# sbyrnes321/metalens

Hardware: AMD Instinct MI355X
Metric: aperture x far-field pair-evals/sec (higher is better)
Workload: dtype f64; 1 GPU; 1 mm dia NA=0.5 lens, lambda=580 nm, 4096x4096 aperture window at pitch lambda/2.2 -> 512x512 far-field directions (bins of the aperture FFT lattice x 1), fp64, on-axis x-dipole at the focus; aperture=4096, farfield=512, rings=197, centre_cells=1219855, orders=survey, pmc_key=gpus=1,aperture=4096,farfield=512,precision=f64,method=auto,zoom=1,pols=1, pmc_stale=True

## Files before the change

### metalens_amd/csrc/nearfield_simple.hip

```cpp
#include <algorithm>
#include <type_traits>

#include "nearfield_math.h"
#include "synth_staging.h"

namespace ml {


#ifdef __HIP_DEVICE_COMPILE__
#define ML_GLOBAL __attribute__((address_space(1)))
#else
#define ML_GLOBAL
#endif
struct Consts {
    double kvac, kvac2, kg2, efh, sx, sy, dz, dz2, z2;
    double b0, b1, b2, b3;
    const ML_GLOBAL double2 *ring_rec, *rot_table, *ring_tab, *premod;
    const ML_GLOBAL int2 *geo_ix;
    ML_GLOBAL double *fields, *partial_power;
    int plane_wave, patches_x, n_rings, outside_is_zero, nx, ny, n_partials;
    double hcoef, pcoef, pol[3];
};
template <bool FIXED3>
__device__ __forceinline__ void load_consts(const NfArgs &a, Consts &K) {
    K.kvac = a.p.kvac;
    K.kvac2 = a.p.kvac2;
    K.kg2 = a.p.k_glass2;
    K.efh = a.e_from_h;
    K.sx = a.p.source_x;
    K.sy = a.p.source_y;
    K.dz = a.p.dz;
    K.dz2 = a.p.dz2;
    K.z2 = a.p.source_z2;
    K.ring_rec = (const ML_GLOBAL double2 *)a.ring_rec;
    K.rot_table = (const ML_GLOBAL double2 *)a.rot_table;
    K.ring_tab = (const ML_GLOBAL double2 *)a.ring_tab;
    K.plane_wave = FIXED3 ? 0 : a.p.plane_wave;
    K.b0 = a.ring_bounds_all[0];
    K.b1 = a.ring_bounds_all[1];
    K.b2 = a.ring_bounds_all[2];
    K.b3 = a.ring_bounds_all[3];
    K.premod = FIXED3 ? nullptr : (const ML_GLOBAL double2 *)a.premod;
    K.geo_ix = (const ML_GLOBAL int2 *)a.geo_ix;
    K.fields = (ML_GLOBAL double *)a.fields;
    K.patches_x = a.patches_x;
    K.n_rings = a.n_rings;
    K.outside_is_zero = a.outside_is_zero;
    K.nx = a.nx;
    K.ny = a.ny;
    if (FIXED3)
        asm volatile("" : "+s"(K.kvac), "+s"(K.kvac2), "+s"(K.kg2), "+s"(K.efh), "+s"(K.sx), "+s"(K.sy), "+s"(K.dz), "+s"(K.dz2),
                     "+s"(K.z2), "+s"(K.ring_rec), "+s"(K.rot_table), "+s"(K.ring_tab));
    else
        asm volatile("" : "+s"(K.kvac), "+s"(K.kvac2), "+s"(K.kg2), "+s"(K.efh), "+s"(K.sx), "+s"(K.sy), "+s"(K.dz), "+s"(K.dz2),
                     "+s"(K.z2), "+s"(K.ring_rec), "+s"(K.rot_table), "+s"(K.ring_tab), "+s"(K.plane_wave));
    K.partial_power = (ML_GLOBAL double *)a.partial_power;
    K.n_partials = a.n_partials;
    K.hcoef = a.hcoef[0];
    K.pcoef = a.pcoef[0];
    K.pol[0] = a.pol[0][0];
    K.pol[1] = a.pol[0][1];
    K.pol[2] = a.pol[0][2];
    if (FIXED3)
        asm volatile("" : "+s"(K.b0), "+s"(K.b1), "+s"(K.b2), "+s"(K.b3), "+s"(K.geo_ix), "+s"(K.fields),
                     "+s"(K.patches_x), "+s"(K.n_rings), "+s"(K.outside_is_zero), "+s"(K.nx), "+s"(K.ny));
    else
        asm volatile("" : "+s"(K.b0), "+s"(K.b1), "+s"(K.b2), "+s"(K.b3), "+s"(K.premod), "+s"(K.geo_ix), "+s"(K.fields),
                     "+s"(K.patches_x), "+s"(K.n_rings), "+s"(K.outside_is_zero), "+s"(K.nx), "+s"(K.ny));
    asm volatile("" : "+s"(K.partial_power), "+s"(K.n_partials), "+s"(K.hcoef), "+s"(K.pcoef), "+s"(K.pol[0]), "+s"(K.pol[1]),
                 "+s"(K.pol[2]));
}

__device__ __forceinline__ void wave_power_k(const NfArgs &a, const Consts &K, double power_here, int bx, int by, int member) {
    power_here = dpp_add<0x111, 0xf>(power_here);
    power_here = dpp_add<0x112, 0xf>(power_here);
    power_here = dpp_add<0x114, 0xf>(power_here);
    power_here = dpp_add<0x118, 0xf>(power_here);
    const int lane = threadIdx.x & 63;
    if ((lane & 15) == 15)
        K.partial_power[(size_t)member * K.n_partials + ((size_t)by * K.patches_x + bx) * 4 + (lane >> 4)] = power_here;
    if (blockIdx.x == 0 && blockIdx.y == 0 && member == 0)
        for (int k = threadIdx.x; k < a.n_viol_keys; k += 64) a.viol_next[k] = 0ull;
}

struct AccS {
    double Exr, Exi, Eyr, Eyi, Hxr, Hxi, Hyr, Hyi;
};

struct OrderShared {
    double kx0, G, ky, ky2;
    c2 E0, X;
};

struct OrderFactors {
    double cxy, cxx, cyy;
    c2 ph;
};

__device__ __forceinline__ double small_int_as_double(int ox) {
    const unsigned m = (unsigned)(ox < 0 ? -ox : ox);
    unsigned hi = m ? 0x3ff00000u + (((0x98640u >> (4 * (m - 1))) & 15u) << 18) : 0u;
    hi |= ox < 0 ? 0x80000000u : 0u;
    return __longlong_as_double((long long)((unsigned long long)hi << 32));
}

struct OrderWalk {
    c2 ph;
    double kx;
};
__device__ __forceinline__ void walk_start(OrderWalk &w, const OrderShared &S, int lo) {
    w.ph = S.E0;
#pragma nounroll
    for (int l = lo; l < 0; ++l) w.ph = cmulf_conj(w.ph, S.X);
#pragma nounroll
    for (int l = 0; l < lo; ++l) w.ph = cmulf(w.ph, S.X);
    w.kx = fma(small_int_as_double(lo), S.G, S.kx0);
}
__device__ __forceinline__ void walk_step(OrderWalk &w, const OrderShared &S) {
    w.ph = cmulf(w.ph, S.X);
    w.kx += S.G;
}

__device__ __forceinline__ bool order_setup(const OrderShared &S, const Consts &K, double kx, double &kt2) {
    kt2 = kx * kx + S.ky2;
    return kt2 <= K.kvac2;
}
__device__ __forceinline__ void order_factors_s(OrderFactors &f, const OrderShared &S, const Consts &K, const OrderWalk &w,
                                                double kt2) {
    const double g = K.efh * rsqrt_fast(K.kg2 - kt2);
    f.cxy = (w.kx * S.ky) * g;
    f.cxx = (K.kg2 - w.kx * w.kx) * g;
    f.cyy = (S.ky2 - K.kg2) * g;
    f.ph = w.ph;
}

__device__ __forceinline__ void order_accumulate(AccS &acc, const OrderFactors &f, double ufy_r, double ufy_i,
                                                 double ufx_r, double ufx_i) {
    const double vy_r = fma(ufy_r, f.ph.r, -(ufy_i * f.ph.i)), vy_i = fma(ufy_r, f.ph.i, ufy_i * f.ph.r);
    const double vx_r = fma(ufx_r, f.ph.r, -(ufx_i * f.ph.i)), vx_i = fma(ufx_r, f.ph.i, ufx_i * f.ph.r);
    acc.Hxr += vy_r;
    acc.Hxi += vy_i;
    acc.Hyr += vx_r;
    acc.Hyi += vx_i;
    acc.Exr = fma(f.cxx, vx_r, fma(f.cxy, vy_r, acc.Exr));
    acc.Exi = fma(f.cxx, vx_i, fma(f.cxy, vy_i, acc.Exi));
    acc.Eyr = fma(-f.cxy, vx_r, fma(f.cyy, vy_r, acc.Eyr));
    acc.Eyi = fma(-f.cxy, vx_i, fma(f.cyy, vy_i, acc.Eyi));
}

template <int NP, int STRIDE>
__device__ __forceinline__ void order_simple(AccS *acc, const double2 *blk, const double *wa, const double *wb,
                                             const double *Hwx, const double *Hwy, const OrderShared &S,
                                             const Consts &K, const OrderWalk &w, bool mine) {
    double kt2;
    if (!((int)order_setup(S, K, w.kx, kt2) & (int)mine)) return;
    OrderFactors f;
    order_factors_s(f, S, K, w, kt2);
    if (NP == 1) {
        double ufy_r, ufy_i, ufx_r, ufx_i;
#pragma unroll
        for (int c = 0; c < 4; ++c) {
            const double2 v0 = blk[(c * 4 + 0) * STRIDE], v1 = blk[(c * 4 + 1) * STRIDE];
            const double2 v2 = blk[(c * 4 + 2) * STRIDE], v3 = blk[(c * 4 + 3) * STRIDE];
            if (c == 0) {
                ufy_r = wa[0] * v0.x;
                ufy_i = wa[0] * v0.y;
                ufx_r = wa[0] * v1.x;
                ufx_i = wa[0] * v1.y;
            } else {
                ufy_r = fma(wa[c], v0.x, ufy_r);
                ufy_i = fma(wa[c], v0.y, ufy_i);
                ufx_r = fma(wa[c], v1.x, ufx_r);
                ufx_i = fma(wa[c], v1.y, ufx_i);
            }
            ufy_r = fma(wb[c], v2.x, ufy_r);
            ufy_i = fma(wb[c], v2.y, ufy_i);
            ufx_r = fma(wb[c], v3.x, ufx_r);
            ufx_i = fma(wb[c], v3.y, ufx_i);
            if (c == 1) __builtin_amdgcn_sched_barrier(0);
        }
        order_accumulate(acc[0], f, ufy_r, ufy_i, ufx_r, ufx_i);
    } else {
        double ar[4], ai[4];
#pragma unroll
        for (int c = 0; c < 4; ++c)
#pragma unroll
            for (int q = 0; q < 4; ++q) {
                const double2 v = blk[(c * 4 + q) * STRIDE];
                ar[q] = c == 0 ? wa[0] * v.x : fma(wa[c], v.x, ar[q]);
                ai[q] = c == 0 ? wa[0] * v.y : fma(wa[c], v.y, ai[q]);
            }
#pragma unroll
        for (int m = 0; m < NP; ++m)
            order_accumulate(acc[m], f, fma(Hwx[m], ar[0], Hwy[m] * ar[2]), fma(Hwx[m], ai[0], Hwy[m] * ai[2]),
                             fma(Hwx[m], ar[1], Hwy[m] * ar[3]), fma(Hwx[m], ai[1], Hwy[m] * ai[3]));
    }
}

__device__ __forceinline__ void locate_uniform(const double *ax, double lim0, double lim1, double u, double v,
                                               int &i0, double &t0, int &i1, double &t1) {
    const double a0 = (u - ax[0]) * ax[2], a1 = (v - ax[3]) * ax[5];
    const double f0 = fmin(fmax(floor(a0), 0.0), lim0), f1 = fmin(fmax(floor(a1), 0.0), lim1);
    i0 = (int)f0;
    i1 = (int)f1;
    t0 = a0 - f0;
    t1 = a1 - f1;
}

__device__ __forceinline__ void locate_axis(const double *axis, int n, double x, int &i, double &t) {
    i = 0;
    for (int a = 1; a < n - 1; ++a) i = (axis[a] <= x) ? a : i;
    const double lo = axis[i], hi = axis[i + 1];
    t = (x - lo) * recip(hi - lo);
}

template <bool RING>
__device__ __forceinline__ void report_orders(const NfArgs &a, double kvac2, double kx0, double G, double ky, int n_slots,
                                              int lo, unsigned present, int slot, double u, double v, double period) {
    const TableDesc &T = RING ? a.tables[slot] : a.center_desc;
    const double ky2 = ky * ky;
    for (int oc = 0; oc < n_slots; ++oc) {
        if (!((present >> oc) & 1u)) continue;
        const double kx = fma((double)(lo + oc), G, kx0);
        if (kx * kx + ky2 <= kvac2) check_bounds(a, T, slot, __popc(present & ((1u << oc) - 1u)), u, v, period, RING);
    }
}

__device__ __forceinline__ void store_fields_k(const Consts &K, int member, int i, int j, c2 Ex, c2 Ey, c2 Hx, c2 Hy) {
    const size_t plane = (size_t)K.nx * K.ny;
    const size_t at = (size_t)i * K.ny + j;
    typedef double double2v __attribute__((ext_vector_type(2)));
    double2v *F = reinterpret_cast<double2v *>(K.fields) + (size_t)member * 4 * plane;
    __builtin_nontemporal_store((double2v){Ex.r, Ex.i}, F + at);
    __builtin_nontemporal_store((double2v){Ey.r, Ey.i}, F + plane + at);
    __builtin_nontemporal_store((double2v){Hx.r, Hx.i}, F + 2 * plane + at);
    __builtin_nontemporal_store((double2v){Hy.r, Hy.i}, F + 3 * plane + at);
}

__device__ __forceinline__ void incidence(const Consts &K, double x, double y, double &ux, double &uy, double &uz,
                                          double &inv) {
    const double dx = x - K.sx, dy = y - K.sy;
    inv = rsqrt_fast(fma(dx, dx, fma(dy, dy, K.dz2)));
    ux = dx * inv;
    uy = dy * inv;
    uz = K.dz * inv;
}

__device__ __forceinline__ void rotate_dir(double ux, double uy, double2 cs, double &uxp, double &uyp) {
    uxp = fma(ux, cs.x, uy * cs.y);
    uyp = fma(uy, cs.x, -(ux * cs.y));
}

__device__ __forceinline__ unsigned lds_address(const double2 *p) {
    return (unsigned)(__UINTPTR_TYPE__)(__attribute__((address_space(3))) const char *)(const char *)p;
}
#pragma clang diagnostic push
#pragma clang diagnostic ignored "-Winline-asm"
template <int N16>
__device__ __forceinline__ void stage_block(const double2 *src, const double2 *lds, unsigned lane_off) {
    const char *base = reinterpret_cast<const char *>(src);
    const unsigned dst = lds_address(lds);
#pragma unroll
    for (int m = 0; m < N16; ++m)
        asm volatile("s_mov_b32 m0, %2\n\ts_nop 0\n\tglobal_load_lds_dwordx4 %0, %1"
                     :
                     : "v"(lane_off), "s"(base + m * 1024), "s"(dst + m * 1024)
                     : "memory", "m0");
}
#pragma clang diagnostic pop

template <int LEFT>
__device__ __forceinline__ void staged_wait() {
    asm volatile("s_waitcnt vmcnt(%0)" ::"n"(LEFT) : "memory");
}

constexpr int CB = CENTER_BLOCK;

typedef int int2v __attribute__((ext_vector_type(2)));

#ifdef ML_PHASE_TIMERS
constexpr int PHASE_SLOTS = 10, PHASE_WAVES = 1 << 18;
__device__ unsigned long long g_phase[(size_t)PHASE_SLOTS * PHASE_WAVES];
#define ML_MARK(k, dep)                                   \
    do {                                                  \
        asm volatile("" ::"v"(dep));                      \
        __builtin_amdgcn_sched_barrier(0);                \
        stamp[k] = __builtin_amdgcn_s_memtime();          \
        __builtin_amdgcn_sched_barrier(0);                \
    } while (0)
#else
#define ML_MARK(k, dep)
#endif

enum { PART_RING = 1, PART_CENTRE = 2 };
#ifndef ML_NF_PRIO
#define ML_NF_PRIO 1
#endif
#define ML_PRIO_AT(point, level)                                                                                          \
    do {                                                                                                                  \
        if (PART == PART_RING && NP == 1 && LISTED && ML_NF_PRIO == 1 && ((point) == 0 || (point) == 2))                  \
            __builtin_amdgcn_s_setprio(level);                                                                            \
    } while (0)
#ifndef ML_NF_KEEP_ROT
#define ML_NF_KEEP_ROT 0
#endif

constexpr int FIXED3_SLOTS = 3, FIXED3_PRESENT = 7;
static_assert(narrow_pitch(FIXED3_SLOTS) == 49 && narrow_cap(narrow_pitch(FIXED3_SLOTS)) == SK_SLOTS_NARROW && FIXED3_SLOTS * UNIT == 48,
              "the fixed-shape ring kernel's pitch, capacity and staging lanes");
template <int NP, int PART, bool LISTED, bool WIDE, bool FIXED3 = false>
__device__ __forceinline__ void synthesize_patch(const NfArgs &a, double2 *s_tab, double2 *s_tab1, int bx, int by) {
    static_assert(!FIXED3 || (NP == 1 && LISTED && !WIDE), "fixed-shape kernels: one source, from the lists, narrow");
    const int lane = threadIdx.x;
    const unsigned lane_off = (unsigned)lane * 16u;
    ML_PRIO_AT(0, 3);
    Consts K;
    load_consts<FIXED3>(a, K);
    const int i = by * 8 + (lane >> 3);
    const int j = bx * 8 + (lane & 7);
    const bool inb = j < K.ny && i < K.nx;
    const double x = a.x_pts[min(i, K.nx - 1)], y = a.y_pts[min(j, K.ny - 1)];
    const int2v ix = reinterpret_cast<const int2v *>(K.geo_ix + ((size_t)by * K.patches_x + bx) * 64)[lane];
#ifdef ML_PHASE_TIMERS
    unsigned long long stamp[PHASE_SLOTS] = {0};
    stamp[0] = __builtin_amdgcn_s_memtime();
    struct StampOut {
        unsigned long long *st;
        size_t wid;
        __device__ ~StampOut() {
            st[7] = __builtin_amdgcn_s_memtime();
            __builtin_amdgcn_s_waitcnt(0);
            st[8] = __builtin_amdgcn_s_memtime();
            if (threadIdx.x == 0 && wid < PHASE_WAVES && PART == PART_RING)
                for (int k = 0; k < PHASE_SLOTS; ++k) g_phase[wid * PHASE_SLOTS + k] = st[k];
        }
    } stamp_out{stamp, (size_t)by * K.patches_x + bx};
#endif
    double ux = 0.0, uy = 0.0, uz = 1.0;
    double Hx_i[NP], Hy_i[NP], power_in[NP];
    if (K.plane_wave) {
#pragma unroll
        for (int m = 0; m < NP; ++m) {
            Hx_i[m] = a.pw_Hx[m];
            Hy_i[m] = a.pw_Hy[m];
            power_in[m] = a.pw_power[m];
        }
    } else {
        double inv;
        incidence(K, x, y, ux, uy, uz, inv);
        const double t = uz * inv, rs = rsqrt_fast(uz);
        const double t2 = t * t;
#pragma unroll
        for (int m = 0; m < NP; ++m) {
            const double *pol = NP == 1 ? K.pol : a.pol[m];
            const double amp = ((NP == 1 ? K.hcoef : a.hcoef[m]) * rs) * t;
            const double hx = fma(uy, pol[2], -(uz * pol[1]));
            const double hy = fma(uz, pol[0], -(ux * pol[2]));
            const double hz = fma(ux, pol[1], -(uy * pol[0]));
            Hx_i[m] = hx * amp;
            Hy_i[m] = hy * amp;
            power_in[m] = ((NP == 1 ? K.pcoef : a.pcoef[m]) * t2) * fma(hx, hx, fma(hy, hy, hz * hz));
        }
    }
    int idx = inb ? ix.x : K.n_rings + 1;
    const int aux = inb ? ix.y : -1;
    ML_MARK(1, idx + aux);
    const int cell_type = idx >> REC_TYPE_SHIFT;
    idx &= (1 << REC_TYPE_SHIFT) - 1;
    const bool lens = idx <= K.n_rings;
    const bool peri_any = lens && idx >= 1;
    const bool peri = PART == PART_RING ? peri_any && (((WIDE ? a.wide_mask : a.narrow_mask) >> cell_type) & 1) != 0 : peri_any;
    const bool mine_too = PART == PART_RING ? (!WIDE || !a.narrow_exists || (LISTED && !a.first_pass && !__ballot(peri_any && ((a.narrow_mask >> cell_type) & 1))))
                                            : (LISTED && (FIXED3 || !a.first_pass) && !__ballot(peri_any));
    if (mine_too) {
#pragma unroll
        for (int m = 0; m < NP; ++m) wave_power_k(a, K, lens ? power_in[m] : 0.0, bx, by, m);
        if (!LISTED && inb && !lens && !K.outside_is_zero) {
            const c2 zero = {0.0, 0.0};
#pragma unroll
            for (int m = 0; m < NP; ++m) store_fields_k(K, m, i, j, zero, zero, zero, zero);
        }
    }
    ML_MARK(2, Hx_i[0]);

    if (PART == PART_CENTRE) {
        if (!__ballot(lens && !peri_any)) return;
    const bool cen = lens && !peri_any && aux >= 0;
    AccS acc[NP];
#pragma unroll
    for (int m = 0; m < NP; ++m) acc[m] = {0, 0, 0, 0, 0, 0, 0, 0};
    const TableDesc &T = a.center_desc;
    int i0, i1;
    double t0, t1;
    if (FIXED3 || T.uniform) {
        locate_uniform(T.uni_ax, (double)(T.n0 - 2), (double)(T.n1 - 2), ux, uy, i0, t0, i1, t1);
    } else {
        locate_axis(T.axis0, T.n0, ux, i0, t0);
        locate_axis(T.axis1, T.n1, uy, i1, t1);
    }
    const bool out_c = (int)(ux < T.bounds[0]) | (int)(ux > T.bounds[1]) | (int)(uy < T.bounds[2]) |
                       (int)(uy > T.bounds[3]);
    const int n2 = T.n2, groups = (n2 + SK_TYPES - 1) / SK_TYPES;
    const int which = min(cell_type, n2 - 1);
    const int grp = which / SK_TYPES;
    const int cblk = (i0 * (T.n1 - 1) + i1) * groups + grp;
    const size_t order_blocks = (size_t)(T.n0 - 1) * (T.n1 - 1) * groups;
    const int n_slots = a.center_n_slots;
    OrderShared S;
    double wa[4], wb[4];
    if (cen) {
        const double2 cc = a.cxy[aux];
        const double ox_ = x - cc.x, oy_ = y - cc.y;
        S.kx0 = K.kvac * ux;
        S.ky = K.kvac * uy;
        double a0 = S.kx0 * ox_ + S.ky * oy_;
        int kq = 0;
        if (!K.plane_wave) {
            const double gx = cc.x - K.sx, gy = cc.y - K.sy;
            const double air = sqrt_exact(gx * gx + gy * gy + K.z2);
            double r;
            reduce_pio2(K.kvac * air, r, kq);
            a0 = r + a0;
        }
        sincos_cw_q(a0, kq, S.E0.i, S.E0.r);
        S.G = T.center_g[0];
        sincos_cw(S.G * ox_, S.X.i, S.X.r);
        S.ky2 = S.ky * S.ky;
        const double w[4] = {(1 - t0) * (1 - t1), (1 - t0) * t1, t0 * (1 - t1), t0 * t1};
#pragma unroll
        for (int c = 0; c < 4; ++c) {
            wa[c] = NP == 1 ? w[c] * Hy_i[0] : w[c];
            wb[c] = NP == 1 ? w[c] * Hx_i[0] : 0.0;
        }
    }
    const int mine_off = which - grp * SK_TYPES;
    unsigned long long todo = __ballot(cen);
    while (todo) {
        const int kl = __builtin_amdgcn_readlane(cblk, __ffsll((long long)todo) - 1);
        const bool mine = cen && cblk == kl;
        todo &= ~__ballot(mine);
        const double2 *src = a.center_tab + (size_t)(unsigned)kl * CB;
        stage_block<CB / 64>(src, s_tab, lane_off);
        OrderShared R = S;
        asm volatile("" : "+v"(R.kx0));
        OrderWalk W;
        walk_start(W, R, a.center_lo);
        if constexpr (FIXED3) {
            const double2 *next = src;
#pragma unroll
            for (int oc = 0; oc < FIXED3_SLOTS; ++oc) {
                const double2 *cur = (oc & 1) ? s_tab1 : s_tab;
                if (oc + 1 < FIXED3_SLOTS) {
                    next += order_blocks * CB;
                    stage_block<CB / 64>(next, (oc & 1) ? s_tab : s_tab1, lane_off);
                    staged_wait<CB / 64>();
                } else {
                    staged_wait<0>();
                }
                order_simple<NP, SK_TYPES>(acc, cur + mine_off, wa, wb, Hy_i, Hx_i, R, K, W, mine);
                if (oc + 1 < FIXED3_SLOTS) walk_step(W, R);
                __builtin_amdgcn_sched_barrier(0);
            }
            continue;
        }
#pragma nounroll
        for (int oc = 0; oc < n_slots; ++oc) {
            const double2 *cur = (oc & 1) ? s_tab1 : s_tab;
            if (oc + 1 < n_slots) {
                stage_block<CB / 64>(src + (size_t)(oc + 1) * order_blocks * CB, (oc & 1) ? s_tab : s_tab1, lane_off);
                staged_wait<CB / 64>();
            } else {
                staged_wait<0>();
            }
            if ((a.center_present >> oc) & 1) order_simple<NP, SK_TYPES>(acc, cur + mine_off, wa, wb, Hy_i, Hx_i, R, K, W, mine);
            walk_step(W, R);
            __builtin_amdgcn_sched_barrier(0);
        }
    }
    if (__ballot(cen && out_c)) {
        if (cen && out_c)
            report_orders<false>(a, K.kvac2, K.kvac * ux, T.center_g[0], K.kvac * uy, a.center_n_slots, a.center_lo,
                                 (unsigned)a.center_present, MAX_SLOTS, ux, uy, 0.0);
    }
    if (cen && K.premod) {
        const double2 t2 = K.premod[j];
        const c2 e = {t2.x, t2.y};
#pragma unroll
        for (int m = 0; m < NP; ++m) {
            AccS &q = acc[m];
            const c2 Ex = cmulf({q.Exr, q.Exi}, e), Ey = cmulf({q.Eyr, q.Eyi}, e);
            const c2 Hx = cmulf({q.Hxr, q.Hxi}, e), Hy = cmulf({q.Hyr, q.Hyi}, e);
            q = {Ex.r, Ex.i, Ey.r, Ey.i, Hx.r, Hx.i, Hy.r, Hy.i};
        }
    }

        if (lens && !peri_any) {
#pragma unroll
            for (int m = 0; m < NP; ++m)
                store_fields_k(K, m, i, j, {acc[m].Exr, acc[m].Exi}, {acc[m].Eyr, acc[m].Eyi},
                             {acc[m].Hxr, acc[m].Hxi}, {acc[m].Hyr, acc[m].Hyi});
        }
        return;
    }
    if (!__ballot(peri)) return;

    double2 r0, r1, cs;
    if (peri) {
        const double2 *rr = K.ring_rec + (size_t)(idx - 1) * 2;
        r0 = rr[0];
        r1 = rr[1];
        cs = K.rot_table[aux];
    }
    double uxp, uyp, t0, t1, xp, yp;
    int cell = 0;
    int c_cur = -1, ns = 1, lo = 0;
    unsigned present = 0;
    bool several = false;
    if (peri) {
        ML_MARK(3, cs.x + r0.x + r1.x);
        xp = x * cs.x + y * cs.y - r0.x;
        yp = -x * cs.y + y * cs.x;
        rotate_dir(ux, uy, cs, uxp, uyp);
    }
    for (unsigned long long pm = __ballot(peri); pm;) {
        const int c0 = __builtin_amdgcn_readlane(cell_type, __ffsll((long long)pm) - 1);
        const bool mc = peri && cell_type == c0;
        pm &= ~__ballot(mc);
        const CollDesc &C = a.coll[c0];
        double ax0 = C.uni_ax[0], ax2 = C.uni_ax[2], ax3 = C.uni_ax[3], ax5 = C.uni_ax[5], lim0 = C.lim0, lim1 = C.lim1;
        int flags = 1, n1m1 = C.n1 - 1, c_ns = FIXED3_SLOTS, c_lo = C.ox_lo, c_present = FIXED3_PRESENT;
        if constexpr (FIXED3) {
            asm volatile("" : "+s"(ax0), "+s"(ax2), "+s"(ax3), "+s"(ax5), "+s"(lim0), "+s"(lim1), "+s"(n1m1), "+s"(c_lo));
        } else {
            flags = C.flags, c_ns = C.n_slots, c_present = C.present;
            asm volatile("" : "+s"(ax0), "+s"(ax2), "+s"(ax3), "+s"(ax5), "+s"(lim0), "+s"(lim1), "+s"(flags), "+s"(n1m1),
                         "+s"(c_ns), "+s"(c_lo), "+s"(c_present));
        }
        if (c_cur < 0) {
            c_cur = c0;
            ns = c_ns;
            lo = c_lo;
            present = (unsigned)c_present;
        } else {
            several = true;
        }
        if (mc) {
            int i0, i1;
            if (flags & 1) {
                const double uni[6] = {ax0, 0.0, ax2, ax3, 0.0, ax5};
                locate_uniform(uni, lim0, lim1, uxp, uyp, i0, t0, i1, t1);
            } else {
                const TableDesc &T = a.tables[a.gc[idx - 1]];
                locate_axis(T.axis0, T.n0, uxp, i0, t0);
                locate_axis(T.axis1, T.n1, uyp, i1, t1);
            }
            asm("v_mad_u32_u24 %0, %1, %2, %3" : "=v"(cell) : "v"(i0), "s"(n1m1), "v"(i1));
            if constexpr (FIXED3)
                cell *= FIXED3_SLOTS;
            else
                asm("v_mul_u32_u24 %0, %1, %2" : "=v"(cell) : "v"(cell), "s"(c_ns));
        }
    }
    const int blk = peri ? (int)(__double_as_longlong(r1.y) & 0x7fffffffll) + cell : -1;
    bool outside = false;
    if (peri) {
        outside = (int)(uxp < K.b0) | (int)(uxp > K.b1) | (int)(uyp < K.b2) | (int)(uyp > K.b3) |
                  (int)((__double_as_longlong(r1.y) >> 32) & 1);
        if (outside) {
            const double *b = a.tables[a.gc[idx - 1]].bounds;
            const double period = r0.y;
            outside = (int)(uxp < b[0]) | (int)(uxp > b[1]) | (int)(uyp < b[2]) | (int)(uyp > b[3]) |
                      (int)(period < b[4]) | (int)(period > b[5]);
        }
    }
    unsigned long long todo = __ballot(peri && cell_type == c_cur);
    unsigned coll_done = 1u << (c_cur & 31);
    int myslot, n_blocks, upp, pitch;
    constexpr int NSLOT = WIDE ? SK_SLOTS : SK_SLOTS_NARROW;
    int lead[NSLOT];
    constexpr int SMALL_SLOTS = SIMPLE_NARROW_SLOTS;
    const int small_pitch = FIXED3 ? narrow_pitch(FIXED3_SLOTS) : a.narrow_pitch, small_cap = FIXED3 ? SK_SLOTS_NARROW : a.narrow_cap;
    auto match = [&]() {
        myslot = -1;
        n_blocks = 0;
        unsigned long long rest = todo;
#pragma unroll
        for (int s = 0; s < NSLOT; ++s) {
            lead[s] = -1;
            if (rest && (WIDE || s < small_cap)) {
                const int kl = __builtin_amdgcn_readlane(blk, __ffsll((long long)rest) - 1);
                const bool mine = blk == kl;
                if (mine) myslot = s;
                rest &= ~__ballot(mine);
                lead[s] = kl;
                n_blocks = s + 1;
            }
        }
        todo = rest;
    };
    auto stage = [&](int s0) {
        const int len = min(upp, ns - s0) * UNIT;
#pragma unroll
        for (int m = 0; m * 64 < UNIT * SIMPLE_MAX_SLOTS; ++m)
            if (m * 64 < len && lane < len - m * 64) {
#pragma unroll
                for (int s = 0; s < NSLOT; ++s)
                    if (lead[s] >= 0)
                        stage_block<1>(K.ring_tab + (size_t)(unsigned)(lead[s] + s0) * UNIT + m * 64,
                                       s_tab + s * pitch + m * 64, lane_off);
            }
    };
    auto begin_round = [&](auto small) {
        match();
        if constexpr (decltype(small)::value) {
            if (lane < (FIXED3 ? FIXED3_SLOTS : ns) * UNIT) {
#pragma unroll
                for (int s = 0; s < NSLOT; ++s)
                    if (lead[s] >= 0)
                        stage_block<1>(K.ring_tab + (size_t)(unsigned)lead[s] * UNIT, s_tab + s * small_pitch, lane_off);
            }
        } else {
            upp = __builtin_amdgcn_readfirstlane(min(ns, (int)((UPP_TABLE >> (4 * (n_blocks - 1))) & 15u)));
            pitch = upp * UNIT + 1;
            stage(0);
        }
    };
    ML_MARK(9, blk);
    begin_round(std::integral_constant<bool, !WIDE>());
    ML_MARK(6, myslot);
    ML_PRIO_AT(2, 0);
    OrderShared S;
    double wa[4], wb[4], Hw_x[NP], Hw_y[NP];
    if (peri) {
        S.kx0 = K.kvac * uxp;
        S.ky = K.kvac * uyp;
        double a0 = S.kx0 * xp + S.ky * yp;
        int kq = 0;
        if (!K.plane_wave) {
            const double rcen = r0.x;
            const double gx = rcen * cs.x - K.sx, gy = rcen * cs.y - K.sy;
            const double air = sqrt_exact(gx * gx + gy * gy + K.z2);
            double r;
            reduce_pio2(K.kvac * air, r, kq);
            a0 = r + a0;
        }
        sincos_cw_q(a0, kq, S.E0.i, S.E0.r);
        S.G = r1.x;
        sincos_cw(S.G * xp, S.X.i, S.X.r);
        S.ky2 = S.ky * S.ky;
        const double w[4] = {(1 - t0) * (1 - t1), (1 - t0) * t1, t0 * (1 - t1), t0 * t1};
#pragma unroll
        for (int m = 0; m < NP; ++m) {
            Hw_y[m] = fma(Hx_i[m], cs.x, Hy_i[m] * cs.y);
            Hw_x[m] = fma(Hy_i[m], cs.x, -(Hx_i[m] * cs.y));
        }
#pragma unroll
        for (int c = 0; c < 4; ++c) {
            wa[c] = NP == 1 ? w[c] * Hw_x[0] : w[c];
            wb[c] = NP == 1 ? w[c] * Hw_y[0] : 0.0;
        }
    }
    AccS pr[NP];
#pragma unroll
    for (int m = 0; m < NP; ++m) pr[m] = {0, 0, 0, 0, 0, 0, 0, 0};
    ML_MARK(4, wa[0] + pr[0].Exr);
    auto finish_round = [&](auto small) {
        OrderShared R = S;
        asm volatile("" : "+v"(R.kx0));
        OrderWalk W;
        walk_start(W, R, lo);
        const bool mine = myslot >= 0;
        if constexpr (FIXED3) {
            const double2 *b = s_tab + max(myslot, 0) * narrow_pitch(FIXED3_SLOTS);
            staged_wait<0>();
#pragma unroll
            for (int sl = 0; sl < FIXED3_SLOTS; ++sl) {
                if (sl) {
                    walk_step(W, R);
                    asm volatile("" : "+v"(W.ph.r), "+v"(W.ph.i), "+v"(W.kx));
                }
                order_simple<NP, 1>(pr, b + sl * UNIT, wa, wb, Hw_x, Hw_y, R, K, W, mine);
                __builtin_amdgcn_sched_barrier(0);
            }
        } else if constexpr (decltype(small)::value) {
            int boff;
            asm("v_mul_u32_u24 %0, %1, %2" : "=v"(boff) : "v"(max(myslot, 0)), "s"(small_pitch));
            const double2 *b = s_tab + boff;
            staged_wait<0>();
#pragma unroll
            for (int sl = 0; sl < SMALL_SLOTS; ++sl) {
                if (sl < ns) {
                    if (sl) {
                        walk_step(W, R);
                        asm volatile("" : "+v"(W.ph.r), "+v"(W.ph.i), "+v"(W.kx));
                    }
                    if ((present >> sl) & 1u) order_simple<NP, 1>(pr, b + sl * UNIT, wa, wb, Hw_x, Hw_y, R, K, W, mine);
                    __builtin_amdgcn_sched_barrier(0);
                }
            }
        } else {
            int boff;
            asm("v_mul_u32_u24 %0, %1, %2" : "=v"(boff) : "v"(max(myslot, 0)), "s"(pitch));
            const double2 *b = s_tab + boff;
            for (int s0 = 0;;) {
                staged_wait<0>();
                const int cnt = min(upp, ns - s0);
#pragma nounroll
                for (int sl = 0; sl < cnt; ++sl) {
                    if ((present >> (s0 + sl)) & 1u) order_simple<NP, 1>(pr, b + sl * UNIT, wa, wb, Hw_x, Hw_y, R, K, W, mine);
                    walk_step(W, R);
                    __builtin_amdgcn_sched_barrier(0);
                }
                s0 += upp;
                if (s0 >= ns) break;
                stage(s0);
            }
        }
    };
    while (true) {
        finish_round(std::integral_constant<bool, !WIDE>());
        if (!todo) {
            if (!several) break;
            const unsigned long long later = __ballot(peri && !((coll_done >> cell_type) & 1u));
            if (!later) break;
            c_cur = __builtin_amdgcn_readlane(cell_type, __ffsll((long long)later) - 1);
            coll_done |= 1u << c_cur;
            if (!FIXED3) ns = a.coll[c_cur].n_slots;
            lo = a.coll[c_cur].ox_lo;
            if (!FIXED3) present = (unsigned)a.coll[c_cur].present;
            todo = __ballot(peri && cell_type == c_cur);
        }
        __builtin_amdgcn_sched_barrier(0);
        begin_round(std::integral_constant<bool, !WIDE>());
    }
    ML_MARK(5, pr[0].Exr + pr[0].Hyi);
    if (__ballot(outside)) {
        if (outside) {
            const int2v ix = reinterpret_cast<const int2v *>(K.geo_ix + ((size_t)by * K.patches_x + bx) * 64)[lane];
            const int ring = (ix.x & ((1 << REC_TYPE_SHIFT) - 1)) - 1;
            const CollDesc *C = a.coll + (ix.x >> REC_TYPE_SHIFT);
            double vx = 0.0, vy = 0.0, vz, vinv, vxp, vyp;
            if (!K.plane_wave) incidence(K, a.x_pts[i], a.y_pts[j], vx, vy, vz, vinv);
            rotate_dir(vx, vy, K.rot_table[ix.y], vxp, vyp);
            const double2 *rr = K.ring_rec + (size_t)ring * 2;
            report_orders<true>(a, K.kvac2, K.kvac * vxp, rr[1].x, K.kvac * vyp, C->n_slots, C->ox_lo, (unsigned)C->present,
                                a.gc[ring], vxp, vyp, rr[0].y);
        }
    }
    if (peri) {
        double2 cs2 = cs;
        if (!(ML_NF_KEEP_ROT && NP == 1)) cs2 = K.rot_table[aux];
        const double cosr = cs2.x, sinr = cs2.y;
        c2 e = {1.0, 0.0};
        if (K.premod) {
            const double2 t2 = K.premod[j];
            e = {t2.x, t2.y};
        }
#pragma unroll
        for (int m = 0; m < NP; ++m) {
            AccS q = pr[m];
            if (K.premod) {
                const c2 Ex = cmulf({q.Exr, q.Exi}, e), Ey = cmulf({q.Eyr, q.Eyi}, e);
                const c2 Hx = cmulf({q.Hxr, q.Hxi}, e), Hy = cmulf({q.Hyr, q.Hyi}, e);
                q = {Ex.r, Ex.i, Ey.r, Ey.i, Hx.r, Hx.i, Hy.r, Hy.i};
            }
            const c2 Ex = {fma(q.Exr, cosr, -(q.Eyr * sinr)), fma(q.Exi, cosr, -(q.Eyi * sinr))};
            const c2 Ey = {fma(q.Exr, sinr, q.Eyr * cosr), fma(q.Exi, sinr, q.Eyi * cosr)};
            const c2 Hx = {fma(q.Hxr, cosr, -(q.Hyr * sinr)), fma(q.Hxi, cosr, -(q.Hyi * sinr))};
            const c2 Hy = {fma(q.Hxr, sinr, q.Hyr * cosr), fma(q.Hxi, sinr, q.Hyi * cosr)};
            store_fields_k(K, m, i, j, Ex, Ey, Hx, Hy);
        }
    }
}

#ifndef ML_NF_RING_MINW
#define ML_NF_RING_MINW 5
#endif

template <int NP, bool LISTED, bool WIDE, bool FIXED3 = false>
__global__ __launch_bounds__(64, NP == 1 ? ML_NF_RING_MINW : 3) void nearfield_ring_kernel(const int2 *list, const NfArgs a) {
    __shared__ double2 s_tab[WIDE ? RING_LDS : RING_LDS_NARROW];
    int bx = blockIdx.x, by = blockIdx.y;
    if (LISTED) {
        if (!FIXED3 && a.list_count && (int)blockIdx.x >= *a.list_count) return;
        const int2 pb = list[blockIdx.x];
        bx = pb.x;
        by = pb.y;
    }
    synthesize_patch<NP, PART_RING, LISTED, WIDE, FIXED3>(a, s_tab, s_tab, bx, by);
}

template <int NP, bool LISTED, bool FIXED3 = false>
__global__ __launch_bounds__(64, 3) void nearfield_centre_kernel(const int2 *list, const NfArgs a) {
    __shared__ double2 s_tab[CB], s_tab1[CB];
    int bx = blockIdx.x, by = blockIdx.y;
    if (LISTED) {
        if (!FIXED3 && a.list_count && (int)blockIdx.x >= *a.list_count) return;
        const int2 pb = list[blockIdx.x];
        bx = pb.x;
        by = pb.y;
    }
    synthesize_patch<NP, PART_CENTRE, LISTED, false, FIXED3>(a, s_tab, s_tab1, bx, by);
}

#ifdef ML_PHASE_TIMERS
extern "C" int ml_debug_phase_dump(unsigned long long *dst, size_t n_waves) {
    return (int)hipMemcpyFromSymbol(dst, HIP_SYMBOL(g_phase), n_waves * PHASE_SLOTS * sizeof(unsigned long long), 0,
                                    hipMemcpyDeviceToHost);
}
#endif

template <int NP>
static int launch_parts(ml_ctx *ctx, const NfArgs &a) {
    const dim3 full((a.ny + 7) / 8, (a.nx + 7) / 8);
    const bool narrow = a.narrow_exists != 0, wide = a.wide_mask != 0;
    if (!a.use_active) {
        NfArgs c = a;
        c.first_pass = 1;
        if (narrow || !wide)
            hipLaunchKernelGGL((nearfield_ring_kernel<NP, false, false>), full, dim3(64), 0, ctx->stream, nullptr, a);
        else
            hipLaunchKernelGGL((nearfield_ring_kernel<NP, false, true>), full, dim3(64), 0, ctx->stream, nullptr, a);
        if (narrow && wide) {
            c.list_count = a.active_count + (size_t)3 * a.count_stride;
            hipLaunchKernelGGL((nearfield_ring_kernel<NP, true, true>), dim3(full.x * full.y), dim3(64), 0, ctx->stream,
                               a.active_list + (size_t)3 * a.list_stride, c);
        }
        c.list_count = a.active_count + (size_t)2 * a.count_stride;
        const int centre_grid = std::min<long>((long)full.x * full.y, a.centre_patch_bound);
        if (centre_grid > 0 && !a.centre_general)
            hipLaunchKernelGGL((nearfield_centre_kernel<NP, true>), dim3(centre_grid), dim3(64), 0, ctx->stream,
                               a.active_list + (size_t)2 * a.list_stride, c);
        ctx->out.ring_form = narrow ? 1 : 0;
        ctx->out.centre_form = centre_grid > 0 && !a.centre_general ? 1 : 0;
        if (a.general_mask || a.centre_general) {
            c.list_count = a.active_count;
            c.use_active = 1;
            ML_TRY(nearfield_general_listed_launch(ctx, c, (int)(full.x * full.y)));
        }
    } else {
        const bool listed = a.use_active && !a.first_pass;
        bool ring_fixed = false, centre_fixed = false;
        if constexpr (NP == 1) {
            ring_fixed = listed && (a.fixed3 & 1) != 0;
            centre_fixed = listed && (a.fixed3 & 2) != 0;
        }
        if (a.n_active[1] > 0) {
            if constexpr (NP == 1) {
                if (ring_fixed)
                    hipLaunchKernelGGL((nearfield_ring_kernel<1, true, false, true>), dim3(a.n_active[1]), dim3(64), 0, ctx->stream,
                                       a.active_list + (size_t)1 * a.list_stride, a);
            }
            if (!ring_fixed)
                hipLaunchKernelGGL((nearfield_ring_kernel<NP, true, false>), dim3(a.n_active[1]), dim3(64), 0, ctx->stream,
                                   a.active_list + (size_t)1 * a.list_stride, a);
        }
        if (a.n_active[3] > 0)
            hipLaunchKernelGGL((nearfield_ring_kernel<NP, true, true>), dim3(a.n_active[3]), dim3(64), 0, ctx->stream,
                               a.active_list + (size_t)3 * a.list_stride, a);
        if (a.n_active[2] > 0) {
            if constexpr (NP == 1) {
                if (centre_fixed)
                    hipLaunchKernelGGL((nearfield_centre_kernel<1, true, true>), dim3(a.n_active[2]), dim3(64), 0, ctx->stream,
                                       a.active_list + (size_t)2 * a.list_stride, a);
            }
            if (!centre_fixed)
                hipLaunchKernelGGL((nearfield_centre_kernel<NP, true>), dim3(a.n_active[2]), dim3(64), 0, ctx->stream,
                                   a.active_list + (size_t)2 * a.list_stride, a);
        }
        ctx->out.ring_form = a.n_active[1] > 0 ? (ring_fixed ? 2 : 1) : 0;
        ctx->out.centre_form = a.n_active[2] > 0 ? (centre_fixed ? 2 : 1) : 0;
        if ((a.general_mask || a.centre_general) && a.n_active[0] > 0)
            ML_TRY(nearfield_general_listed_launch(ctx, a, a.n_active[0]));
    }
    ML_HIP(hipGetLastError());
    return ML_OK;
}

int nearfield_simple_launch(ml_ctx *ctx, const NfArgs &a) {
    return a.n_pol == 1 ? launch_parts<1>(ctx, a) : a.n_pol == 2 ? launch_parts<2>(ctx, a) : launch_parts<3>(ctx, a);
}

}
```

### metalens_amd/csrc/synth_staging.h

```cpp
#pragma once

#include "lens_pack.h"

namespace ml {

constexpr int SK_SLOTS = 6;
#ifndef ML_RING_LDS_WIDE
#define ML_RING_LDS_WIDE 448
#endif
constexpr int SK_SLOTS_NARROW = 8;
constexpr int RING_LDS_NARROW = SK_SLOTS_NARROW * (3 * UNIT + 1), RING_LDS = ML_RING_LDS_WIDE;
static_assert(SK_SLOTS * (SIMPLE_NARROW_SLOTS * UNIT + 1) <= RING_LDS_NARROW, "six blocks of four orders fit");
constexpr int narrow_pitch(int narrow_slots_max) { return UNIT * narrow_slots_max + 1; }
constexpr int narrow_cap(int pitch) { return RING_LDS_NARROW / pitch < SK_SLOTS_NARROW ? RING_LDS_NARROW / pitch : SK_SLOTS_NARROW; }
static_assert(narrow_cap(narrow_pitch(3)) == SK_SLOTS_NARROW && narrow_cap(narrow_pitch(SIMPLE_NARROW_SLOTS)) == SK_SLOTS,
              "eight blocks of three orders, six of four");
constexpr unsigned slots_per_pass(int n) { return (unsigned)((RING_LDS / n - 1) / UNIT < 15 ? (RING_LDS / n - 1) / UNIT : 15); }
constexpr unsigned UPP_TABLE = slots_per_pass(1) | slots_per_pass(2) << 4 | slots_per_pass(3) << 8 | slots_per_pass(4) << 12 |
                               slots_per_pass(5) << 16 | slots_per_pass(6) << 20;
static_assert(slots_per_pass(SK_SLOTS) >= 1, "block buffer too small");
constexpr int SK_TYPES = 20;
static_assert(SK_TYPES == CENTER_GROUP, "the centre table's cell blocks hold groups of SK_TYPES types");

constexpr int NF_SLOTS = 6;
constexpr int NF_CHUNK = 4;

}
```

Baseline: 9731000 billion pair-evals/s.

## Stage centre table in half-blocks to halve LDS and raise occupancy

The centre kernel now double-buffers half-blocks (two interpolation nodes each) instead of whole cell blocks. It interleaves staging of the next halves with the node accumulation of the current ones, and computes the order factors before waiting on the loads. Shared memory per workgroup is halved, and the launch-bounds minimum waves for NP==1 rises from 3 to 5 so more waves can be resident. The trade-off is more waits and finer synchronisation per order, plus possible register pressure from the tighter bound.

```diff
diff --git a/metalens_amd/csrc/nearfield_simple.hip b/metalens_amd/csrc/nearfield_simple.hip
--- a/metalens_amd/csrc/nearfield_simple.hip
+++ b/metalens_amd/csrc/nearfield_simple.hip
@@ -197,6 +197,58 @@
     }
 }
 
+template <int NP>
+struct NodeSums {
+    double r[NP == 1 ? 2 : 4], i[NP == 1 ? 2 : 4];
+};
+template <int NP, int STRIDE, int C0>
+__device__ __forceinline__ void order_nodes(NodeSums<NP> &u, const double2 *pair, const double *wa, const double *wb) {
+    if (NP == 1) {
+#pragma unroll
+        for (int c = C0; c < C0 + 2; ++c) {
+            const double2 *nd = pair + (c - C0) * 4 * STRIDE;
+            const double2 v0 = nd[0 * STRIDE], v1 = nd[1 * STRIDE];
+            const double2 v2 = nd[2 * STRIDE], v3 = nd[3 * STRIDE];
+            if (c == 0) {
+                u.r[0] = wa[0] * v0.x;
+                u.i[0] = wa[0] * v0.y;
+                u.r[1] = wa[0] * v1.x;
+                u.i[1] = wa[0] * v1.y;
+            } else {
+                u.r[0] = fma(wa[c], v0.x, u.r[0]);
+                u.i[0] = fma(wa[c], v0.y, u.i[0]);
+                u.r[1] = fma(wa[c], v1.x, u.r[1]);
+                u.i[1] = fma(wa[c], v1.y, u.i[1]);
+            }
+            u.r[0] = fma(wb[c], v2.x, u.r[0]);
+            u.i[0] = fma(wb[c], v2.y, u.i[0]);
+            u.r[1] = fma(wb[c], v3.x, u.r[1]);
+            u.i[1] = fma(wb[c], v3.y, u.i[1]);
+        }
+    } else {
+#pragma unroll
+        for (int c = C0; c < C0 + 2; ++c)
+#pragma unroll
+            for (int q = 0; q < 4; ++q) {
+                const double2 v = pair[((c - C0) * 4 + q) * STRIDE];
+                u.r[q] = c == 0 ? wa[0] * v.x : fma(wa[c], v.x, u.r[q]);
+                u.i[q] = c == 0 ? wa[0] * v.y : fma(wa[c], v.y, u.i[q]);
+            }
+    }
+}
+template <int NP>
+__device__ __forceinline__ void order_finish(AccS *acc, const OrderFactors &f, const NodeSums<NP> &u, const double *Hwx,
+                                             const double *Hwy) {
+    if (NP == 1) {
+        order_accumulate(acc[0], f, u.r[0], u.i[0], u.r[1], u.i[1]);
+    } else {
+#pragma unroll
+        for (int m = 0; m < NP; ++m)
+            order_accumulate(acc[m], f, fma(Hwx[m], u.r[0], Hwy[m] * u.r[2]), fma(Hwx[m], u.i[0], Hwy[m] * u.i[2]),
+                             fma(Hwx[m], u.r[1], Hwy[m] * u.r[3]), fma(Hwx[m], u.i[1], Hwy[m] * u.i[3]));
+    }
+}
+
 __device__ __forceinline__ void locate_uniform(const double *ax, double lim0, double lim1, double u, double v,
                                                int &i0, double &t0, int &i1, double &t1) {
     const double a0 = (u - ax[0]) * ax[2], a1 = (v - ax[3]) * ax[5];
@@ -275,6 +327,19 @@
 }
 
 constexpr int CB = CENTER_BLOCK;
+constexpr int HB = CENTRE_HALF;
+
+__device__ __forceinline__ void stage_half(const double2 *src, const double2 *lds, unsigned lane_off) {
+    stage_block<CENTRE_HALF_LOADS - 1>(src, lds, lane_off);
+    if (lane_off < CENTRE_HALF_TAIL * 16u)
+        stage_block<1>(src + (CENTRE_HALF_LOADS - 1) * 64, lds + (CENTRE_HALF_LOADS - 1) * 64, lane_off);
+}
+__device__ __forceinline__ void staged_wait_half(int k, int n) {
+    if (centre_half_step(k, n).wait)
+        staged_wait<CENTRE_HALF_LOADS>();
+    else
+        staged_wait<0>();
+}
 
 typedef int int2v __attribute__((ext_vector_type(2)));
 
@@ -435,29 +500,43 @@
     }
     const int mine_off = which - grp * SK_TYPES;
     unsigned long long todo = __ballot(cen);
+    unsigned long long out_lanes = __ballot(cen && out_c);
+    asm volatile("" : "+s"(out_lanes));
     while (todo) {
         const int kl = __builtin_amdgcn_readlane(cblk, __ffsll((long long)todo) - 1);
         const bool mine = cen && cblk == kl;
         todo &= ~__ballot(mine);
         const double2 *src = a.center_tab + (size_t)(unsigned)kl * CB;
-        stage_block<CB / 64>(src, s_tab, lane_off);
+        static_assert(CENTRE_PROLOGUE_HALVES == 2 && CENTRE_BUFFERS == 2, "the round's first two halves, one per buffer");
+        stage_half(src, s_tab, lane_off);
+        stage_half(src + HB, s_tab1, lane_off);
         OrderShared R = S;
         asm volatile("" : "+v"(R.kx0));
         OrderWalk W;
         walk_start(W, R, a.center_lo);
+        auto order_halves = [&](int oc, int n, bool present) {
+            const double2 *next = src + (size_t)(oc + 1) * order_blocks * CB;
+            double kt2;
+            const bool act = present && ((int)order_setup(R, K, W.kx, kt2) & (int)mine) != 0;
+            OrderFactors f;
+            NodeSums<NP> u;
+            if (act) order_factors_s(f, R, K, W, kt2);
+            staged_wait_half(2 * oc, n);
+            if (act) order_nodes<NP, SK_TYPES, 0>(u, s_tab + mine_off, wa, wb);
+            __builtin_amdgcn_sched_barrier(0);
+            if (centre_half_step(2 * oc, n).stage_next >= 0) stage_half(next, s_tab, lane_off);
+            staged_wait_half(2 * oc + 1, n);
+            if (act) {
+                order_nodes<NP, SK_TYPES, 2>(u, s_tab1 + mine_off, wa, wb);
+                order_finish<NP>(acc, f, u, Hy_i, Hx_i);
+            }
+            __builtin_amdgcn_sched_barrier(0);
+            if (centre_half_step(2 * oc + 1, n).stage_next >= 0) stage_half(next + HB, s_tab1, lane_off);
+        };
         if constexpr (FIXED3) {
-            const double2 *next = src;
 #pragma unroll
             for (int oc = 0; oc < FIXED3_SLOTS; ++oc) {
-                const double2 *cur = (oc & 1) ? s_tab1 : s_tab;
-                if (oc + 1 < FIXED3_SLOTS) {
-                    next += order_blocks * CB;
-                    stage_block<CB / 64>(next, (oc & 1) ? s_tab : s_tab1, lane_off);
-                    staged_wait<CB / 64>();
-                } else {
-                    staged_wait<0>();
-                }
-                order_simple<NP, SK_TYPES>(acc, cur + mine_off, wa, wb, Hy_i, Hx_i, R, K, W, mine);
+                order_halves(oc, FIXED3_SLOTS, true);
                 if (oc + 1 < FIXED3_SLOTS) walk_step(W, R);
                 __builtin_amdgcn_sched_barrier(0);
             }
@@ -465,22 +544,18 @@
         }
 #pragma nounroll
         for (int oc = 0; oc < n_slots; ++oc) {
-            const double2 *cur = (oc & 1) ? s_tab1 : s_tab;
-            if (oc + 1 < n_slots) {
-                stage_block<CB / 64>(src + (size_t)(oc + 1) * order_blocks * CB, (oc & 1) ? s_tab : s_tab1, lane_off);
-                staged_wait<CB / 64>();
-            } else {
-                staged_wait<0>();
-            }
-            if ((a.center_present >> oc) & 1) order_simple<NP, SK_TYPES>(acc, cur + mine_off, wa, wb, Hy_i, Hx_i, R, K, W, mine);
+            order_halves(oc, n_slots, (a.center_present >> oc) & 1);
             walk_step(W, R);
             __builtin_amdgcn_sched_barrier(0);
         }
     }
-    if (__ballot(cen && out_c)) {
-        if (cen && out_c)
-            report_orders<false>(a, K.kvac2, K.kvac * ux, T.center_g[0], K.kvac * uy, a.center_n_slots, a.center_lo,
-                                 (unsigned)a.center_present, MAX_SLOTS, ux, uy, 0.0);
+    if (out_lanes) {
+        if ((out_lanes >> lane) & 1ull) {
+            double vx = 0.0, vy = 0.0, vz, vinv;
+            if (!K.plane_wave) incidence(K, a.x_pts[i], a.y_pts[j], vx, vy, vz, vinv);
+            report_orders<false>(a, K.kvac2, K.kvac * vx, T.center_g[0], K.kvac * vy, a.center_n_slots, a.center_lo,
+                                 (unsigned)a.center_present, MAX_SLOTS, vx, vy, 0.0);
+        }
     }
     if (cen && K.premod) {
         const double2 t2 = K.premod[j];
@@ -776,6 +851,9 @@
 #ifndef ML_NF_RING_MINW
 #define ML_NF_RING_MINW 5
 #endif
+#ifndef ML_NF_CENTRE_MINW
+#define ML_NF_CENTRE_MINW 5
+#endif
 
 template <int NP, bool LISTED, bool WIDE, bool FIXED3 = false>
 __global__ __launch_bounds__(64, NP == 1 ? ML_NF_RING_MINW : 3) void nearfield_ring_kernel(const int2 *list, const NfArgs a) {
@@ -791,8 +869,9 @@
 }
 
 template <int NP, bool LISTED, bool FIXED3 = false>
-__global__ __launch_bounds__(64, 3) void nearfield_centre_kernel(const int2 *list, const NfArgs a) {
-    __shared__ double2 s_tab[CB], s_tab1[CB];
+__global__ __launch_bounds__(64, NP == 1 ? ML_NF_CENTRE_MINW : 3) void nearfield_centre_kernel(const int2 *list, const NfArgs a) {
+    __shared__ double2 s_tab[HB], s_tab1[HB];
+    static_assert(sizeof(double2) * 2 * HB == CENTRE_LDS_BYTES, "the centre kernel's LDS");
     int bx = blockIdx.x, by = blockIdx.y;
     if (LISTED) {
         if (!FIXED3 && a.list_count && (int)blockIdx.x >= *a.list_count) return;
diff --git a/metalens_amd/csrc/synth_staging.h b/metalens_amd/csrc/synth_staging.h
--- a/metalens_amd/csrc/synth_staging.h
+++ b/metalens_amd/csrc/synth_staging.h
@@ -22,6 +22,22 @@
 constexpr int SK_TYPES = 20;
 static_assert(SK_TYPES == CENTER_GROUP, "the centre table's cell blocks hold groups of SK_TYPES types");
 
+constexpr int CENTRE_HALF = CENTER_BLOCK / 2;
+constexpr int CENTRE_HALF_LOADS = (CENTRE_HALF + 63) / 64;
+constexpr int CENTRE_HALF_TAIL = CENTRE_HALF - (CENTRE_HALF_LOADS - 1) * 64;
+constexpr int CENTRE_BUFFERS = 2;
+constexpr int CENTRE_PROLOGUE_HALVES = CENTRE_BUFFERS;
+constexpr int CENTRE_LDS_BYTES = CENTRE_BUFFERS * CENTRE_HALF * 16;
+static_assert(CENTRE_HALF * 2 == CENTER_BLOCK && CENTRE_HALF == 2 * 4 * SK_TYPES, "a half block is two nodes of four amplitudes");
+static_assert(CENTRE_HALF_TAIL > 0 && CENTRE_HALF_TAIL <= 64, "the last load of a half");
+static_assert(CENTRE_LDS_BYTES <= RING_LDS_NARROW * 16, "the centre kernel's LDS stays within the size the ring kernel is measured good at");
+struct CentreHalfStep {
+    int buffer, wait, stage_next;
+};
+constexpr CentreHalfStep centre_half_step(int k, int n_orders) {
+    return {k % CENTRE_BUFFERS, k + 1 < 2 * n_orders ? CENTRE_HALF_LOADS : 0, k + CENTRE_BUFFERS < 2 * n_orders ? k + CENTRE_BUFFERS : -1};
+}
+
 constexpr int NF_SLOTS = 6;
 constexpr int NF_CHUNK = 4;
 
```

Result: no change. 9656000 billion pair-evals/s (-0.8%).
